# cvg/pixel-perfect-sfm

Hardware: AMD Instinct MI355X
Metric: featuremetric residuals+Jacobians evaluated/sec (1M obs) (higher is better)
Workload: dtype f32 horizontal / f64 vertical+normalisation on f16 patches; 1 GPU; BASELINE.json configs[2]: synthetic 200 cams / 200000 points / 1000000 obs featuremetric BA residual+Jacobian evaluation, 128-ch fp16 16x16 patches, SIMPLE_RADIAL, fused six-scalar Jacobian reduction; n_obs=1000000, channels=128, patch=16, obs_per_gpu=1000000, partition=none

## Files before the change

pixel-perfect-sfm_amd/csrc/pxr_ba_gram.hip:

```cpp
#include <hip/hip_runtime.h>

#include <algorithm>

#include "pxr_ba_solve.h"
#include "pxr_device.h"
#include "pxr_gram.h"
#include "pxr_internal.h"

namespace pxr {

constexpr int GC_STRIDE = IG_GDOUBLES + 16;

struct GramArgs {
  pxr_ba_view v;
  const void* arena; const int32_t* corners; const double* scales;
  int H, W, l2_normalize;
  double* G;
  int2* cell;
  int* dirty;
  const double* r2;
  double* rec;
};

template <typename ST, int C>
__global__ __launch_bounds__(64) void k_gram_build(const GramArgs a) {
// ... 26 lines not shown
      if (2 * lane < C) rr = *reinterpret_cast<const double2*>(a.v.d_refs + (size_t)p * C + 2 * lane);
      return j;
    };
    auto build = [&](const GramTexels<ST, C>& tx, const double2& rr, int slot, int j) {
      if (2 * lane < C) *reinterpret_cast<double2*>(&refbuf[slot][2 * lane]) = rr;
      __syncthreads();
      double* g = a.G + (size_t)(base + j) * GC_STRIDE;
      gram_contract<ST, C>(tx, refbuf[slot], g, g + IG_GDOUBLES);
    };
    GramTexels<ST, C> t0, t1, t2;
    int s0 = take(t0, rr0), s1 = take(t1, rr1), s2 = take(t2, rr2);
    while (true) {
      if (s0 < 0) break;
      build(t0, rr0, 0, s0); s0 = take(t0, rr0);
      if (s1 < 0) break;
      build(t1, rr1, 1, s1); s1 = take(t1, rr1);
      if (s2 < 0) break;
      build(t2, rr2, 2, s2); s2 = take(t2, rr2);
    }
  }
}

template <bool FIRST>
__device__ __forceinline__ void gram_eval_eight(const GramArgs& a, double* S, int64_t i, int nq, int lane) {
  const int q = lane >> 3, sub = lane & 7, ri = sub >> 1, ci = 2 * (sub & 1);
  constexpr int NT = (8 * GC_STRIDE / 2 + 63) / 64, PER = GC_STRIDE / 2;
  static_assert(NT * 64 == 8 * PER, "the last request stays inside the buffer");
  const int n2 = nq * PER;
#pragma unroll
  for (int j = 0; j < NT; ++j) {
    const int e = min(lane + 64 * j, n2 - 1);
    const double2* src;
    if (FIRST) {
      src = reinterpret_cast<const double2*>(a.G + (size_t)__shfl((int)i, 0) * GC_STRIDE) + e;
    } else {
      const int64_t oi = __shfl((int)i, 8 * (e / PER));
      src = reinterpret_cast<const double2*>(a.G + (size_t)oi * GC_STRIDE) + e % PER;
    }
    __builtin_amdgcn_global_load_lds((const __attribute__((address_space(1))) void*)src,
                                     (__attribute__((address_space(3))) void*)(S + 2 * 64 * j), 16, 0, 0);
  }
  const int img = a.v.d_obs_image[i];
  const int pt = a.v.d_obs_point[i];
  const int64_t pidx = a.v.d_obs_patch[i];
  int2 cached = make_int2(0, 0);
  if (FIRST) cached = a.cell[i];
  const int cam = a.v.d_image_camera[img];
  double qv[4], t[3], X[3], k[PXR_KPAD];
#pragma unroll
  for (int j = 0; j < 4; ++j) qv[j] = a.v.d_qvec[4 * (size_t)img + j];
#pragma unroll
  for (int j = 0; j < 3; ++j) { t[j] = a.v.d_tvec[3 * (size_t)img + j]; X[j] = a.v.d_xyz[3 * (size_t)pt + j]; }
#pragma unroll
  for (int j = 0; j < PXR_KPAD; ++j) k[j] = a.v.d_cam_params[(size_t)cam * PXR_KPAD + j];
  const double sx = a.scales[2 * pidx], sy = a.scales[2 * pidx + 1];
  const double cx = (double)a.corners[2 * pidx], cy = (double)a.corners[2 * pidx + 1];
  const double r2 = a.r2[pt];
  double x, y;
  world_to_pixel(a.v.d_cam_model[cam], k, qv, t, X, x, y);
  const double u = x * sx - 0.5 - cx, v = y * sy - 0.5 - cy;
  const double rf = floor(v), cf = floor(u);
  const int row = texel_index(rf, a.H), col = texel_index(cf, a.W);
  const bool miss = FIRST && (cached.x != row || cached.y != col);
  if (FIRST && q < nq && sub == 0) {
    a.dirty[i] = miss ? 1 : 0;
    if (miss) a.cell[i] = make_int2(row, col);
  }
  double wu[4], dwu[4], wv[4], dwv[4];
  catmull_rom_weights(u - cf, wu, dwu);
  catmull_rom_weights(v - rf, wv, dwv);
  __builtin_amdgcn_s_waitcnt(0x0f70);
  __syncthreads();
  if (q >= nq || miss) return;
  const double* Gq = S + (size_t)q * GC_STRIDE;
  double ya[3], yb[3];
  gram_rows_times_weights(Gq, sub, wu, dwu, wv, dwv, ya, yb);
  const double2 d2 = *reinterpret_cast<const double2*>(Gq + IG_GDOUBLES + 2 * sub);
  const double wvo = pick4(wv, ri), dwvo = pick4(dwv, ri);
  const double wua = ci == 0 ? wu[0] : wu[2], wub = ci == 0 ? wu[1] : wu[3];
  const double dwua = ci == 0 ? dwu[0] : dwu[2], dwub = ci == 0 ? dwu[1] : dwu[3];
  const double oma = wvo * wua, omb = wvo * wub, omca = wvo * dwua, omcb = wvo * dwub, omra = dwvo * wua, omrb = dwvo * wub;
  const double Sgg = row8_sum(fma(oma, ya[0], omb * yb[0])), Sgc = row8_sum(fma(oma, ya[1], omb * yb[1]));
  const double Sgr = row8_sum(fma(oma, ya[2], omb * yb[2]));
  const double Scc = row8_sum(fma(omca, ya[1], omcb * yb[1])), Scr = row8_sum(fma(omca, ya[2], omcb * yb[2]));
  const double Srr = row8_sum(fma(omra, ya[2], omrb * yb[2]));
  const double Sfd = row8_sum(fma(oma, d2.x, omb * d2.y)), Scd = row8_sum(fma(omca, d2.x, omcb * d2.y));
  const double Srd = row8_sum(fma(omra, d2.x, omrb * d2.y));
  if (sub != 0) return;
  double s, gcc, gcr, grr, bc, br;
  if (a.l2_normalize) {
    const double ninv = 1.0 / sqrt(Sgg), n2inv = ninv * ninv;
    const double pc = Sgc * n2inv, pr = Sgr * n2inv;
    s = 1.0 - 2.0 * Sfd * ninv + r2;
    gcc = (Scc - Sgc * pc) * n2inv; gcr = (Scr - Sgc * pr) * n2inv; grr = (Srr - Sgr * pr) * n2inv;
    bc = -(Scd - Sfd * pc) * ninv; br = -(Srd - Sfd * pr) * ninv;
  } else {
    s = Sgg - 2.0 * Sfd + r2;
    gcc = Scc; gcr = Scr; grr = Srr; bc = Sgc - Scd; br = Sgr - Srd;
  }
  if (s < 0.0) s = 0.0;
  double2* out = reinterpret_cast<double2*>(a.rec + (size_t)i * PXR_OBS_REC);
  out[0] = make_double2(s, gcc * sx * sx);
  out[1] = make_double2(gcr * sx * sy, grr * sy * sy);
  out[2] = make_double2(bc * sx, br * sy);
  out[3] = make_double2(x, y);
}

__global__ __launch_bounds__(64) void k_gram_eval(const GramArgs a) {
  __shared__ __align__(16) double S[8 * GC_STRIDE];
  const int lane = threadIdx.x;
  const int64_t o0 = (int64_t)blockIdx.x * 8;
  const int nq = (int)min<int64_t>(8, a.v.n_obs - o0);
  if (nq <= 0) return;
  gram_eval_eight<true>(a, S, o0 + min(lane >> 3, nq - 1), nq, lane);
}

__global__ __launch_bounds__(64) void k_gram_eval_dirty(const GramArgs a) {
  __shared__ __align__(16) double S[8 * GC_STRIDE];
  const int lane = threadIdx.x;
  const int64_t base = (int64_t)blockIdx.x * 64, n = a.v.n_obs;
  unsigned long long todo = __ballot(base + lane < n && a.dirty[min(base + lane, n - 1)] != 0);
#pragma clang loop unroll(disable)
  while (todo != 0ull) {
    const int nq = min(8, __popcll(todo));
    unsigned long long m = todo;
    for (int t = min(lane >> 3, nq - 1); t > 0; --t) m &= m - 1ull;
    const int64_t i = base + __ffsll((long long)m) - 1;
    gram_eval_eight<false>(a, S, i, nq, lane);
    for (int t = 0; t < nq; ++t) todo &= todo - 1ull;
    __syncthreads();
  }
}

__global__ __launch_bounds__(256) void k_gram_count_dirty(int64_t n, const int* __restrict__ dirty, int* __restrict__ count) {
  const int64_t i = (int64_t)blockIdx.x * blockDim.x + threadIdx.x;
  const unsigned long long m = __ballot(i < n && dirty[min(i, n - 1)] != 0);
  if ((threadIdx.x & 63) == 0 && m != 0ull) atomicAdd(count, __popcll(m));
}

__global__ __launch_bounds__(256) void k_gram_r2(int64_t n_pts, int C, const double* __restrict__ refs, double* __restrict__ r2) {
  const int64_t t = (int64_t)blockIdx.x * blockDim.x + threadIdx.x;
  const int64_t p = t >> 4;
  const int sub = (int)(t & 15);
  double acc = 0.0;
  if (p < n_pts)
    for (int ch = sub; ch < C; ch += 16) { const double d = refs[(size_t)p * C + ch]; acc = fma(d, d, acc); }
  acc = row16_sum(acc);
  if (p < n_pts && sub == 0) r2[p] = acc;
}

__global__ __launch_bounds__(256) void k_gram_invalidate(int64_t n, int2* __restrict__ cell) {
  const int64_t i = (int64_t)blockIdx.x * blockDim.x + threadIdx.x;
  if (i < n) cell[i] = make_int2(-1000000, -1000000);
}
// ... 30 lines not shown
  }
  gram_layout(ctx->d_gram, n, np, out, &need);
  hipStream_t st = ctx->stream;
  hipLaunchKernelGGL(k_gram_invalidate, dim3((unsigned)((n + 255) / 256)), dim3(256), 0, st, n, static_cast<int2*>(out->cell));
  hipLaunchKernelGGL(k_gram_r2, dim3((unsigned)((np * 16 + 255) / 256)), dim3(256), 0, st, np, arena->C, view->d_refs, out->r2);
  return hip_check(hipGetLastError(), "Gram-matrix cache set-up");
}

int gram_build_flagged(pxr_ctx* ctx, pxr_arena* arena, const pxr_ba_view* v, const GramCache& gc) {
  GramArgs a;
  a.v = *v;
  a.arena = arena->d_data; a.corners = arena->d_corners; a.scales = arena->d_scales;
  a.H = arena->H; a.W = arena->W; a.l2_normalize = 0;
  a.G = gc.G; a.cell = static_cast<int2*>(gc.cell); a.dirty = gc.list; a.r2 = gc.r2; a.rec = nullptr;
  const int64_t n = v->n_obs;
  const unsigned build_grid = (unsigned)std::min<int64_t>((n + 63) / 64, (int64_t)ctx->num_cus * 16);
#define GRAM_BUILD(ST, CC) hipLaunchKernelGGL((k_gram_build<ST, CC>), dim3(build_grid), dim3(64), 0, ctx->stream, a)
  if (arena->dtype == PXR_F16) { if (arena->C == 128) GRAM_BUILD(_Float16, 128); else GRAM_BUILD(_Float16, 64); }
  else { if (arena->C == 128) GRAM_BUILD(float, 128); else GRAM_BUILD(float, 64); }
#undef GRAM_BUILD
  return hip_check(hipGetLastError(), "Gram-matrix build");
}

int gram_evaluate(pxr_ctx* ctx, pxr_arena* arena, const pxr_ba_view* v, const pxr_interp_cfg* cfg, const GramCache& gc, double* rec) {
  GramArgs a;
  a.v = *v;
  a.arena = arena->d_data; a.corners = arena->d_corners; a.scales = arena->d_scales;
  a.H = arena->H; a.W = arena->W; a.l2_normalize = cfg->l2_normalize;
  a.G = gc.G; a.cell = static_cast<int2*>(gc.cell); a.dirty = gc.list; a.r2 = gc.r2; a.rec = rec;
  hipStream_t st = ctx->stream;
  const int64_t n = v->n_obs;
  hipLaunchKernelGGL(k_gram_eval, dim3((unsigned)((n + 7) / 8)), dim3(64), 0, st, a);
  const unsigned build_grid = (unsigned)std::min<int64_t>((n + 63) / 64, (int64_t)ctx->num_cus * 16);
#define GRAM_BUILD(ST, CC) hipLaunchKernelGGL((k_gram_build<ST, CC>), dim3(build_grid), dim3(64), 0, st, a)
  if (arena->dtype == PXR_F16) { if (arena->C == 128) GRAM_BUILD(_Float16, 128); else GRAM_BUILD(_Float16, 64); }
  else { if (arena->C == 128) GRAM_BUILD(float, 128); else GRAM_BUILD(float, 64); }
#undef GRAM_BUILD
  hipLaunchKernelGGL(k_gram_eval_dirty, dim3((unsigned)((n + 63) / 64)), dim3(64), 0, st, a);
  return hip_check(hipGetLastError(), "Gram-matrix evaluation");
}

}

extern "C" int pxr_ba_eval_gram(pxr_ctx* ctx, pxr_arena* arena, const pxr_ba_view* view, const pxr_interp_cfg* cfg, int reset,
                                double* d_rec, int32_t* h_rebuilt) {
  using namespace pxr;
  PXR_REQUIRE(ctx && arena && view && cfg && d_rec, "pxr_ba_eval_gram: NULL argument");
  PXR_REQUIRE(gram_eval_supported(arena, view), "pxr_ba_eval_gram: needs feature patches of 128 / 64 channels in fp16 / fp32 storage and reference descriptors");
  PXR_HIP(hipSetDevice(ctx->device));
  GramCache gc;
  size_t need = 0;
  gram_layout(ctx->d_gram, view->n_obs, view->n_points, &gc, &need);
  if (reset || ctx->gram_bytes < need) {
    if (int rc = gram_eval_prepare(ctx, arena, view, &gc)) return rc;
  }
  if (int rc = gram_evaluate(ctx, arena, view, cfg, gc, d_rec)) return rc;
  if (h_rebuilt) {
    PXR_HIP(hipMemsetAsync(gc.count, 0, sizeof(int), ctx->stream));
    hipLaunchKernelGGL(k_gram_count_dirty, dim3((unsigned)((view->n_obs + 255) / 256)), dim3(256), 0, ctx->stream, view->n_obs, gc.list, gc.count);
    PXR_HIP(hipMemcpyAsync(h_rebuilt, gc.count, sizeof(int32_t), hipMemcpyDeviceToHost, ctx->stream));
    PXR_HIP(hipStreamSynchronize(ctx->stream));
  }
// ... 4 lines not shown
```

pixel-perfect-sfm_amd/csrc/pxr_ba_solve.h:

```cpp
#pragma once
#include <hip/hip_runtime.h>

#include <functional>

#include "pixsfm_hip.h"

namespace pxr {

struct SolveDev {
  pxr_ba_view v;
  const int* pose_off; const int* pose_dim; const int* tmask;
  const int* intr_off; const int* intr_dim; const int* cmask;
  const int* pt_var;
  const double* scale_c;
  const double* scale_p;
  int n_c; int DC; int LS;
  int ldS;
};

struct ImgChunk { int img; int64_t begin, end; };

__device__ __forceinline__ int col_index(const SolveDev& d, int img, int cam, int a) {
  const int pd = d.pose_dim[img];
  return a < pd ? d.pose_off[img] + a : d.intr_off[cam] + (a - pd);
}

__device__ __forceinline__ void y_row(const double* __restrict__ W, const double* __restrict__ T, int64_t i, int a, int DC,
                                      int64_t pt, double& y0, double& y1, double& y2) {
  const double* Wi = W + ((size_t)i * DC + a) * 3;
  const double* Tp = T + 6 * (size_t)pt;
  const double w0 = Wi[0], w1 = Wi[1], w2 = Wi[2];
  y0 = w0 * Tp[0] + w1 * Tp[1] + w2 * Tp[2];
  y1 = w0 * Tp[1] + w1 * Tp[3] + w2 * Tp[4];
  y2 = w0 * Tp[2] + w1 * Tp[4] + w2 * Tp[5];
}

__device__ __forceinline__ double wave_sum(double v) {
  for (int off = 32; off > 0; off >>= 1) v += __shfl_xor(v, off);
  return v;
}

}
```

pixel-perfect-sfm_amd/csrc/pxr_ba_solve.hip:

```cpp
#include <hip/hip_runtime.h>

#include <algorithm>
#include <chrono>
#include <cmath>
#include <cstdlib>
#include <cstring>
#include <limits>
#include <thread>
#include <vector>

#include "pxr_ba_pcg.h"
#include "pxr_ba_solve.h"
#include "pxr_device.h"
#include "pxr_internal.h"

namespace pxr {


constexpr int JAC_THREADS = 128;

__global__ __launch_bounds__(JAC_THREADS) void k_jac(const SolveDev d, const double* __restrict__ rec,
                                                     pxr_loss loss, double* __restrict__ L, double* __restrict__ W) {
  extern __shared__ double jstage[];
  const int lane = threadIdx.x & 63, wave = threadIdx.x >> 6;
  const int LS = d.LS, W3 = 3 * d.DC, WS = W3 + 1;
  double* Lw = jstage + (size_t)wave * 64 * (LS + WS);
  double* Ww = Lw + (size_t)64 * LS;
  const int64_t i0 = (int64_t)blockIdx.x * blockDim.x + wave * 64;
  const int64_t i = i0 + lane;
  const int n_valid = (int)min((int64_t)64, d.v.n_obs - i0);
  if (i < d.v.n_obs) {
  const int img = d.v.d_obs_image[i], pt = d.v.d_obs_point[i], cam = d.v.d_image_camera[img];
  double q[4], t[3], X[3], k[PXR_KPAD];
#pragma unroll
  for (int j = 0; j < 4; ++j) q[j] = d.v.d_qvec[4 * (size_t)img + j];
#pragma unroll
  for (int j = 0; j < 3; ++j) { t[j] = d.v.d_tvec[3 * (size_t)img + j]; X[j] = d.v.d_xyz[3 * (size_t)pt + j]; }
#pragma unroll
  for (int j = 0; j < PXR_KPAD; ++j) k[j] = d.v.d_cam_params[(size_t)cam * PXR_KPAD + j];
  const int model = d.v.d_cam_model[cam];
  double x, y, A[2][3], Pq[2][4], PX[2][3], Pk[2][PXR_KPAD];
  world_to_pixel_jac(model, k, q, t, X, x, y, A, Pq, PX, Pk);

  const double* r = rec + (size_t)i * PXR_OBS_REC;
  const double s = r[0], gxx = r[1], gxy = r[2], gyy = r[3], bx = r[4], by = r[5];
// ... 51 lines not shown
    for (int a = 0; a < 3; ++a) {
      if ((tm >> a) & 1) continue;
      const double sc = d.scale_c[po + col];
      put(col, A[0][a] * sc, A[1][a] * sc);
      ++col;
    }
  }
  if (d.intr_dim[cam] > 0) {
    const int io = d.intr_off[cam], cm = d.cmask[cam], K = camera_num_params(model);
    int kc = 0;
#pragma unroll
    for (int a = 0; a < PXR_KPAD; ++a) {
      if (a >= K || ((cm >> a) & 1)) continue;
      const double sc = d.scale_c[io + kc];
      put(col, Pk[0][a] * sc, Pk[1][a] * sc);
      ++col; ++kc;
    }
  }
  for (; col < d.DC; ++col) put(col, 0.0, 0.0);
  }
  __threadfence_block();
  __builtin_amdgcn_wave_barrier();
  if (n_valid <= 0) return;
  double* Lg = L + (size_t)i0 * LS;
  for (int x = lane; x < n_valid * LS; x += 64) Lg[x] = Lw[x];
  double* Wg = W + (size_t)i0 * W3;
  for (int x = lane; x < n_valid * W3; x += 64) { const int o = x / W3; Wg[x] = Ww[o * WS + (x - o * W3)]; }
}

__global__ __launch_bounds__(256) void k_point(const SolveDev d, const int64_t* __restrict__ pt_ptr,
                                               const int64_t* __restrict__ pt_obs,
                                               const double* __restrict__ L, double* __restrict__ V,
                                               double* __restrict__ gp) {
  const int64_t p = (int64_t)blockIdx.x * blockDim.x + threadIdx.x;
  if (p >= d.v.n_points) return;
  double v[6] = {0, 0, 0, 0, 0, 0}, g[3] = {0, 0, 0};
  for (int64_t o = pt_ptr[p]; o < pt_ptr[p + 1]; ++o) {
    const double* Lo = L + (size_t)pt_obs[o] * d.LS;
    const double m00 = Lo[0], m01 = Lo[1], m11 = Lo[2], b0 = Lo[3], b1 = Lo[4];
    const double e0[3] = {Lo[5], Lo[6], Lo[7]}, e1[3] = {Lo[8], Lo[9], Lo[10]};
    double me0[3], me1[3];
#pragma unroll
    for (int j = 0; j < 3; ++j) { me0[j] = m00 * e0[j] + m01 * e1[j]; me1[j] = m01 * e0[j] + m11 * e1[j]; }
    v[0] += e0[0] * me0[0] + e1[0] * me1[0];
    v[1] += e0[0] * me0[1] + e1[0] * me1[1];
    v[2] += e0[0] * me0[2] + e1[0] * me1[2];
    v[3] += e0[1] * me0[1] + e1[1] * me1[1];
    v[4] += e0[1] * me0[2] + e1[1] * me1[2];
    v[5] += e0[2] * me0[2] + e1[2] * me1[2];
#pragma unroll
    for (int j = 0; j < 3; ++j) g[j] += e0[j] * b0 + e1[j] * b1;
  }
#pragma unroll
  for (int j = 0; j < 6; ++j) V[6 * p + j] = v[j];
#pragma unroll
  for (int j = 0; j < 3; ++j) gp[3 * p + j] = g[j];
}

constexpr int IMG_BATCH = 128;

__global__ __launch_bounds__(256) void k_img(const SolveDev d, const ImgChunk* __restrict__ chunks,
                                             const int64_t* __restrict__ img_obs,
                                             const double* __restrict__ L, double* __restrict__ U,
                                             double* __restrict__ gc, int block_form, double det_scale,
                                             double* __restrict__ chunk_trace, double* __restrict__ kpart, int ne_max) {
  extern __shared__ double stage[];
  const ImgChunk ch = chunks[blockIdx.x];
  const int img = ch.img, cam = d.v.d_image_camera[img];
  const int dc = d.pose_dim[img] + d.intr_dim[cam];
  if (dc == 0) { if (threadIdx.x == 0 && chunk_trace) chunk_trace[blockIdx.x] = 0.0; return; }
  const int LS = d.LS;
  double* red = stage + (size_t)IMG_BATCH * LS;
  const int NP = dc * (dc + 1) / 2, NE = NP + dc;
  const int slices = 256 / NE;
  const int e = threadIdx.x % NE, sl = threadIdx.x / NE;
  int a = 0, b = 0;
  const bool is_g = e >= NP;
  if (is_g) { a = e - NP; }
  else { int rem = e; a = 0; while (rem >= dc - a) { rem -= dc - a; ++a; } b = a + rem; }
// ... 822 lines not shown
      if (!on || a.wanted <= a.cap) return;
      (void)hipDeviceSynchronize();
      if (ctx->d_solve_arena) (void)hipFree(ctx->d_solve_arena);
      ctx->d_solve_arena = nullptr; ctx->solve_arena_bytes = 0;
      const size_t want = a.wanted + a.wanted / 16 + (1u << 20);
      if (hipMalloc(&ctx->d_solve_arena, want) == hipSuccess) ctx->solve_arena_bytes = want;
      else { (void)hipGetLastError(); ctx->d_solve_arena = nullptr; }
    }
  } arena_scope(ctx);
  const bool setup_verbose = std::getenv("PXR_VERBOSE") != nullptr;
  auto setup_mark = [&](const char* what) {
    if (setup_verbose)
      fprintf(stderr, "[pxr_ba_solve] setup: %-28s at %.2f ms\n", what,
              std::chrono::duration<double, std::milli>(std::chrono::steady_clock::now() - t_setup0).count());
  };
  const int64_t n_obs = view->n_obs, n_pts = view->n_points;
  const int n_img = view->n_images, n_cam = view->n_cameras;

  std::vector<int32_t> obs_image, obs_point, image_camera(n_img), cam_model(n_cam);
  std::vector<int64_t> img_cnt(n_img + 1, 0), pt_cnt;
  DevBuf<unsigned long long> d_cnt;
  DevBuf<int> d_flags;
  bool device_lists = n_img <= SORT_MAX_IMAGES && std::getenv("PXR_BA_SETUP_HOST") == nullptr;
  PXR_HIP(hipMemcpyAsync(image_camera.data(), view->d_image_camera, 4 * n_img, hipMemcpyDeviceToHost, st));
  PXR_HIP(hipMemcpyAsync(cam_model.data(), view->d_cam_model, 4 * n_cam, hipMemcpyDeviceToHost, st));
  setup_mark("camera tables read");
  if (device_lists) {
    int h_flags[2] = {0, 0};
    RC(d_cnt.alloc((size_t)n_img + 1 + (size_t)n_pts + 1 + 1)); RC(d_flags.alloc(2));
    setup_mark("counter buffers");
    PXR_HIP(hipMemsetAsync(d_cnt.p, 0, sizeof(unsigned long long) * d_cnt.n, st));
    PXR_HIP(hipMemsetAsync(d_flags.p, 0, sizeof(int) * 2, st));
    hipLaunchKernelGGL(k_count_indices, dim3((unsigned)((n_obs + COUNT_CHUNK - 1) / COUNT_CHUNK)), dim3(256), sizeof(unsigned int) * n_img, st, n_obs, view->d_obs_image,
                       view->d_obs_point, n_img, n_pts, d_cnt.p, d_cnt.p + n_img + 1, d_flags.p);
    static_assert(sizeof(unsigned long long) == sizeof(int64_t), "counter width");
    PXR_HIP(hipMemcpyAsync(img_cnt.data(), d_cnt.p, sizeof(int64_t) * (n_img + 1), hipMemcpyDeviceToHost, st));
    PXR_HIP(hipMemcpyAsync(h_flags, d_flags.p, sizeof(int) * 2, hipMemcpyDeviceToHost, st));
    PXR_HIP(hipStreamSynchronize(st));
    PXR_REQUIRE(h_flags[0] == 0, "pxr_ba_solve: an observation references an image / point out of range");
    if (h_flags[1]) {
      device_lists = false;
      std::fill(img_cnt.begin(), img_cnt.end(), 0);
    }
  }
  if (!device_lists) {
    pt_cnt.assign(n_pts + 1, 0);
// ... 83 lines not shown
    for (int i = 0; i < n_img; ++i) {
      const int c = image_camera[i];
      const bool joint = cam_users[c] == 1 && intr_dim[c] > 0;
      if (pose_dim[i] == 0 && !joint) continue;
      const int g = open_group();
      add_cols(g, pose_off[i], pose_dim[i]);
      if (joint) add_cols(g, intr_off[c], intr_dim[c]);
    }
    for (int c = 0; c < n_cam; ++c)
      if (cam_users[c] != 1 && intr_dim[c] > 0) add_cols(open_group(), intr_off[c], intr_dim[c]);
    for (int c = 0; c < n_c; ++c) PXR_REQUIRE(col_group[c].x >= 0, "pxr_ba_solve: internal: column %d in no preconditioner block", c);
  }
  setup_mark("host structure (CSR, chunks)");
  DevBuf<int> d_pose_off, d_pose_dim, d_tmask, d_intr_off, d_intr_dim, d_cmask, d_pt_var;
  DevBuf<int64_t> d_img_obs, d_pt_ptr, d_pt_obs;
  DevBuf<ImgChunk> d_chunks, d_schur_chunks;
  DevBuf<int4> d_obs_cols, d_so;
  DevBuf<int> d_part_obs;
  RC(d_pose_off.upload(pose_off, st)); RC(d_pose_dim.upload(pose_dim, st)); RC(d_tmask.upload(tmask, st));
  RC(d_intr_off.upload(intr_off, st)); RC(d_intr_dim.upload(intr_dim, st)); RC(d_cmask.upload(cmask, st));
  RC(d_chunks.upload(chunks, st));
  DevBuf<uint8_t> d_pt_const;
  DevBuf<unsigned long long> d_pt_part;
  unsigned long long h_n_pvar = 0;
  if (!device_lists) { RC(d_pt_var.upload(pt_var, st)); RC(d_pt_ptr.upload(pt_cnt, st)); }
  if (device_lists) {
    const int n_parts = (int)((n_pts + PT_SCAN_CHUNK - 1) / PT_SCAN_CHUNK);
    unsigned long long* const d_pt_cnt = d_cnt.p + n_img + 1;
    RC(d_pt_var.alloc(n_pts)); RC(d_pt_ptr.alloc((size_t)n_pts + 1)); RC(d_pt_const.alloc(n_pts)); RC(d_pt_part.alloc(n_parts));
    PXR_HIP(hipMemcpyAsync(d_pt_const.p, h_point_const, (size_t)n_pts, hipMemcpyHostToDevice, st));
    hipLaunchKernelGGL(k_pt_scan_partials, dim3(n_parts), dim3(256), 0, st, n_pts, (const unsigned long long*)d_pt_cnt, d_pt_part.p);
    hipLaunchKernelGGL(k_pt_scan_apply, dim3(n_parts), dim3(256), 0, st, n_pts, (const unsigned long long*)d_pt_cnt, (const unsigned long long*)d_pt_part.p,
                       (const uint8_t*)d_pt_const.p, d_pt_ptr.p, d_pt_var.p, d_pt_cnt + n_pts + 1);
    PXR_HIP(hipMemcpyAsync(&h_n_pvar, d_pt_cnt + n_pts + 1, sizeof(h_n_pvar), hipMemcpyDeviceToHost, st));
    RC(d_img_obs.alloc(n_obs)); RC(d_pt_obs.alloc(n_obs));
    hipLaunchKernelGGL(k_iota, dim3(nblk(n_obs)), dim3(256), 0, st, n_obs, d_pt_obs.p);
    DevBuf<int64_t> d_img_ptr;
    DevBuf<int> d_hist;
    const int n_chunks = (int)((n_obs + SORT_CHUNK - 1) / SORT_CHUNK);
    RC(d_img_ptr.upload(img_cnt, st)); RC(d_hist.alloc((size_t)n_chunks * n_img));
    hipLaunchKernelGGL(k_sort_hist, dim3(n_chunks), dim3(256), sizeof(int) * n_img, st, n_obs, view->d_obs_image, n_img, d_hist.p);
    hipLaunchKernelGGL(k_sort_offsets, dim3((n_img + 255) / 256), dim3(256), 0, st, n_img, n_chunks, d_img_ptr.p, d_hist.p);
    hipLaunchKernelGGL(k_sort_scatter, dim3(n_chunks), dim3(256), sizeof(int) * (n_img + 256), st, n_obs, view->d_obs_image, n_img,
                       d_hist.p, d_img_obs.p);
    LAUNCH_CHECK("observation-list kernels");
    setup_mark("list kernels launched");
    PXR_HIP(hipStreamSynchronize(st));
    setup_mark("list kernels done");
    n_pvar = (int64_t)h_n_pvar;
    PXR_REQUIRE(n_c > 0 || n_pvar > 0, "pxr_ba_solve: every parameter block is constant");
  } else {
    RC(d_img_obs.upload(img_obs, st)); RC(d_pt_obs.upload(pt_obs, st));
  }
  RC(d_schur_chunks.upload(schur_chunks, st));
  RC(d_obs_cols.alloc(n_obs)); RC(d_so.alloc(n_obs)); RC(d_part_obs.alloc(n_obs));
  hipLaunchKernelGGL(k_build_descriptors, dim3(nblk(n_obs)), dim3(256), 0, st, n_obs, view->d_obs_image, view->d_obs_point,
                     view->d_image_camera, d_pt_obs.p, d_img_obs.p, d_pt_ptr.p, d_pt_var.p, d_pose_off.p, d_pose_dim.p,
                     d_intr_off.p, d_intr_dim.p, d_obs_cols.p, d_part_obs.p, d_so.p);
  LAUNCH_CHECK("k_build_descriptors");
  setup_mark("index uploads");
  const size_t nc1 = n_c ? n_c : 1;
  DevBuf<double> L, V, gp, Vd0, T, W, U, S , gcd , damp_c, scale_c, scale_p,
      delta_c, delta_p, rec_a, rec_b, q1, t1, k1, X1, scal;
  RC(L.alloc((size_t)n_obs * LS)); RC(V.alloc((size_t)n_pts * 6)); RC(gp.alloc((size_t)n_pts * 3));
  RC(Vd0.alloc((size_t)n_pts * 3)); RC(T.alloc((size_t)n_pts * 6));
  RC(W.alloc((size_t)n_obs * DC * 3));
  RC(U.alloc(iterative ? (size_t)n_img * DC * DC : nc1 * nc1)); RC(S.alloc(iterative ? 1 : (nc1 + 1) * (nc1 + 1)));
// ... 138 lines not shown
  RC(chunk_trace.alloc(chunks.size() + 1));
  auto det_scale_for = [](double md, double cost_now) {
    const double bound = 8.0 * std::max({md, std::sqrt(2.0 * md * std::max(cost_now, 0.0)), 1e-300});
    return std::ldexp(1.0, 62 - (int)std::ceil(std::log2(bound)));
  };
  double lin_md = 1.0;
  bool gram_cache = !geom && ctx->gram_cache && gram_eval_supported(arena, view) && cfg->use_float_simd == 0;
  bool gram_inner = !geom && opt->use_inner_iterations != 0 && arena->dtype != PXR_F64 && (arena->C == 128 || arena->C == 64) && !getenv("PXR_INNER_OLD") &&
                    !getenv("PXR_INNER_PACKED") && cfg->use_float_simd == 0;
  for (int c = 0; c < n_cam; ++c) gram_inner = gram_inner && cam_model[c] <= PXR_OPENCV;
  bool inner_cache = gram_inner && gram_eval_supported(arena, view) && !getenv("PXR_INNER_NO_CACHE");
  GramCache gram;
  if ((gram_cache || inner_cache) && gram_eval_prepare(ctx, arena, view, &gram) != PXR_OK) {
    gram_cache = false; inner_cache = false;
    (void)set_error(PXR_OK, "");
  }
  bool geom_ext = false;
  for (int c = 0; c < n_cam; ++c) geom_ext = geom_ext || cam_model[c] > PXR_OPENCV;
  setup_mark("Gram-matrix cache prepared");
  bool gram_warm = false;
  int n_evaluations = 0;
  bool cur_is_exact = true;
  auto evaluate = [&](const pxr_ba_view& v, double* rec) -> int {
    if (geom) RC(geom_eval(ctx, &v, d_obs_xy, rec, nullptr));
    else if (gram_cache && n_evaluations > 0) { RC(gram_evaluate(ctx, arena, &v, cfg, gram, rec)); gram_warm = true; }
    else RC(ba_eval_with_cost(ctx, arena, &v, cfg, 1, rec, nullptr, nullptr, nullptr, nullptr, nullptr));
    ++n_evaluations;
    hipLaunchKernelGGL(k_cost_limbs, dim3(1024), dim3(256), 0, st, (const double*)rec, n_obs, *loss, slimb.p + 0 * PXR_LIMBS);
    LAUNCH_CHECK("cost");
    return PXR_OK;
  };
  double lin_scale = 0.0;
  auto linearize = [&](const double* rec) -> int {
    hipLaunchKernelGGL(k_jac, dim3((unsigned)((n_obs + JAC_THREADS - 1) / JAC_THREADS)), dim3(JAC_THREADS),
                       sizeof(double) * (JAC_THREADS / 64) * 64 * (LS + 3 * DC + 1), st, dv, rec, *loss, L.p, W.p);
    hipLaunchKernelGGL(k_point, dim3(nblk(n_pts)), dim3(256), 0, st, dv, d_pt_ptr.p, d_pt_obs.p, L.p, V.p, gp.p);
    PXR_HIP(hipMemsetAsync(U.p, 0, sizeof(double) * U.n, st));
    PXR_HIP(hipMemsetAsync(gcd.p, 0, sizeof(double) * gcd.n, st));
    if (n_c > 0 && !chunks.empty()) {
      hipLaunchKernelGGL(k_img, dim3((unsigned)chunks.size()), dim3(256), sizeof(double) * ((size_t)IMG_BATCH * LS + 256), st, dv,
                         d_chunks.p, d_img_obs.p, L.p, U.p, gc, iterative ? 1 : 0, lin_scale, lin_scale != 0.0 ? chunk_trace.p : (double*)nullptr,
                         det_iter ? det_kpart.p : (double*)nullptr, det_ne_max);
      if (det_iter) {
        RC(pcg_blocks_from_partials(st, dv, d_kchunk_ptr.p, det_kpart.p, det_ne_max, U.p, det_gimg.p, d_col_ent_ptr.p, d_col_ent.p, diagU, gc));
        LAUNCH_CHECK("linearize kernels");
        RC(ar(gcd.p, 2 * (int64_t)nc1));
        return PXR_OK;
      }
      if (lin_scale != 0.0) {
        hipLaunchKernelGGL(k_diag_and_trace, dim3(1), dim3(1024), 0, st, n_c, (const double*)U.p, diagU, (const double*)chunk_trace.p, (int)chunks.size(),
                           reinterpret_cast<long long*>(gcd.p + 2 * nc1));
        RC(ar_i64(reinterpret_cast<long long*>(gcd.p), 2 * (int64_t)nc1 + PXR_LIMBS));
        hipLaunchKernelGGL(k_finish_and_stats, dim3(1), dim3(1024), 0, st, n_c, 2 * (int)nc1, gcd.p, lin_scale,
                           reinterpret_cast<const long long*>(gcd.p + 2 * nc1), lin_stats.p);
        LAUNCH_CHECK("linearize kernels");
        return PXR_OK;
      }
      if (iterative) RC(pcg_diag_from_blocks(st, dv, U.p, diagU));
      else hipLaunchKernelGGL(k_extract_diag, dim3(nblk(n_c)), dim3(256), 0, st, n_c, U.p, diagU);
// ... 379 lines not shown
```

Measured before the change: 1.467 billion residual_blocks/s.

## Pipeline Gram evaluation, fuse loss cost into eval, and fold point sums into k_jac

Replaces the one-block-per-eight-observations Gram evaluation with a persistent, double-buffered kernel that prefetches the next group's Gram rows and camera/point parameters while the current group is projected and reduced. The robust-loss cost is accumulated inside the evaluation and dirty kernels, so the separate cost pass over the records is no longer launched. Point Hessian and gradient sums for points whose observations all sit in one 64-observation window are computed inside k_jac, and the k_point pass only handles the listed straddling points. The change adds register pressure and extra setup (a straddler list and a host readback), and it assumes the point-ordered observation layout keeps most points inside one window.

```diff
diff --git a/pixel-perfect-sfm_amd/csrc/pxr_ba_gram.hip b/pixel-perfect-sfm_amd/csrc/pxr_ba_gram.hip
--- a/pixel-perfect-sfm_amd/csrc/pxr_ba_gram.hip
+++ b/pixel-perfect-sfm_amd/csrc/pxr_ba_gram.hip
@@ -1,6 +1,8 @@
 #include <hip/hip_runtime.h>
 
 #include <algorithm>
+#include <cstdlib>
+#include <cstring>
 
 #include "pxr_ba_solve.h"
 #include "pxr_device.h"
@@ -73,8 +75,7 @@
 }
 
 template <bool FIRST>
-__device__ __forceinline__ void gram_eval_eight(const GramArgs& a, double* S, int64_t i, int nq, int lane) {
-  const int q = lane >> 3, sub = lane & 7, ri = sub >> 1, ci = 2 * (sub & 1);
+__device__ __forceinline__ void gram_request(const GramArgs& a, double* S, int64_t i, int nq, int lane) {
   constexpr int NT = (8 * GC_STRIDE / 2 + 63) / 64, PER = GC_STRIDE / 2;
   static_assert(NT * 64 == 8 * PER, "the last request stays inside the buffer");
   const int n2 = nq * PER;
@@ -91,38 +92,68 @@
     __builtin_amdgcn_global_load_lds((const __attribute__((address_space(1))) void*)src,
                                      (__attribute__((address_space(3))) void*)(S + 2 * 64 * j), 16, 0, 0);
   }
-  const int img = a.v.d_obs_image[i];
-  const int pt = a.v.d_obs_point[i];
-  const int64_t pidx = a.v.d_obs_patch[i];
-  int2 cached = make_int2(0, 0);
-  if (FIRST) cached = a.cell[i];
-  const int cam = a.v.d_image_camera[img];
-  double qv[4], t[3], X[3], k[PXR_KPAD];
-#pragma unroll
-  for (int j = 0; j < 4; ++j) qv[j] = a.v.d_qvec[4 * (size_t)img + j];
-#pragma unroll
-  for (int j = 0; j < 3; ++j) { t[j] = a.v.d_tvec[3 * (size_t)img + j]; X[j] = a.v.d_xyz[3 * (size_t)pt + j]; }
-#pragma unroll
-  for (int j = 0; j < PXR_KPAD; ++j) k[j] = a.v.d_cam_params[(size_t)cam * PXR_KPAD + j];
-  const double sx = a.scales[2 * pidx], sy = a.scales[2 * pidx + 1];
-  const double cx = (double)a.corners[2 * pidx], cy = (double)a.corners[2 * pidx + 1];
-  const double r2 = a.r2[pt];
-  double x, y;
-  world_to_pixel(a.v.d_cam_model[cam], k, qv, t, X, x, y);
-  const double u = x * sx - 0.5 - cx, v = y * sy - 0.5 - cy;
+}
+
+struct GramObs { int img, pt, cam; int64_t pidx; int2 cached; };
+struct GramParams { double qv[4], t[3], X[3], k[PXR_KPAD], sx, sy, cx, cy, r2; int model; };
+struct GramProj { double x, y, sx, sy, r2, wu[4], dwu[4], wv[4], dwv[4]; bool miss; };
+
+template <bool FIRST>
+__device__ __forceinline__ void gram_load_obs(const GramArgs& a, int64_t i, GramObs& o) {
+  o.img = a.v.d_obs_image[i];
+  o.pt = a.v.d_obs_point[i];
+  o.pidx = a.v.d_obs_patch[i];
+  o.cached = make_int2(0, 0);
+  if (FIRST) o.cached = a.cell[i];
+}
+__device__ __forceinline__ void gram_load_params(const GramArgs& a, const GramObs& o, GramParams& p) {
+#pragma unroll
+  for (int j = 0; j < 4; ++j) p.qv[j] = a.v.d_qvec[4 * (size_t)o.img + j];
+#pragma unroll
+  for (int j = 0; j < 3; ++j) { p.t[j] = a.v.d_tvec[3 * (size_t)o.img + j]; p.X[j] = a.v.d_xyz[3 * (size_t)o.pt + j]; }
+#pragma unroll
+  for (int j = 0; j < PXR_KPAD; ++j) p.k[j] = a.v.d_cam_params[(size_t)o.cam * PXR_KPAD + j];
+  p.sx = a.scales[2 * o.pidx]; p.sy = a.scales[2 * o.pidx + 1];
+  p.cx = (double)a.corners[2 * o.pidx]; p.cy = (double)a.corners[2 * o.pidx + 1];
+  p.r2 = a.r2[o.pt];
+  p.model = a.v.d_cam_model[o.cam];
+}
+
+__device__ __forceinline__ void gram_copy_params(GramParams& d, const GramParams& p) {
+#pragma unroll
+  for (int j = 0; j < 4; ++j) d.qv[j] = p.qv[j];
+#pragma unroll
+  for (int j = 0; j < 3; ++j) { d.t[j] = p.t[j]; d.X[j] = p.X[j]; }
+#pragma unroll
+  for (int j = 0; j < PXR_KPAD; ++j) d.k[j] = p.k[j];
+  d.sx = p.sx; d.sy = p.sy; d.cx = p.cx; d.cy = p.cy; d.r2 = p.r2; d.model = p.model;
+}
+
+template <bool FIRST>
+__device__ __forceinline__ void gram_project(const GramArgs& a, int64_t i, int nq, int lane, int2 cached, const GramParams& p,
+                                             GramProj& pr) {
+  const int q = lane >> 3, sub = lane & 7;
+  world_to_pixel(p.model, p.k, p.qv, p.t, p.X, pr.x, pr.y);
+  const double u = pr.x * p.sx - 0.5 - p.cx, v = pr.y * p.sy - 0.5 - p.cy;
   const double rf = floor(v), cf = floor(u);
   const int row = texel_index(rf, a.H), col = texel_index(cf, a.W);
-  const bool miss = FIRST && (cached.x != row || cached.y != col);
+  pr.miss = FIRST && (cached.x != row || cached.y != col);
   if (FIRST && q < nq && sub == 0) {
-    a.dirty[i] = miss ? 1 : 0;
-    if (miss) a.cell[i] = make_int2(row, col);
-  }
-  double wu[4], dwu[4], wv[4], dwv[4];
-  catmull_rom_weights(u - cf, wu, dwu);
-  catmull_rom_weights(v - rf, wv, dwv);
-  __builtin_amdgcn_s_waitcnt(0x0f70);
-  __syncthreads();
-  if (q >= nq || miss) return;
+    a.dirty[i] = pr.miss ? 1 : 0;
+    if (pr.miss) a.cell[i] = make_int2(row, col);
+  }
+  catmull_rom_weights(u - cf, pr.wu, pr.dwu);
+  catmull_rom_weights(v - rf, pr.wv, pr.dwv);
+  pr.sx = p.sx; pr.sy = p.sy; pr.r2 = p.r2;
+}
+
+__device__ __forceinline__ bool gram_record(const GramArgs& a, const double* S, int64_t i, int nq, int lane, const GramProj& pr,
+                                            double& s_out) {
+  const int q = lane >> 3, sub = lane & 7, ri = sub >> 1, ci = 2 * (sub & 1);
+  s_out = 0.0;
+  if (q >= nq || pr.miss) return false;
+  const double (&wu)[4] = pr.wu; const double (&dwu)[4] = pr.dwu; const double (&wv)[4] = pr.wv; const double (&dwv)[4] = pr.dwv;
+  const double sx = pr.sx, sy = pr.sy, r2 = pr.r2, x = pr.x, y = pr.y;
   const double* Gq = S + (size_t)q * GC_STRIDE;
   double ya[3], yb[3];
   gram_rows_times_weights(Gq, sub, wu, dwu, wv, dwv, ya, yb);
@@ -137,14 +168,14 @@
   const double Srr = row8_sum(fma(omra, ya[2], omrb * yb[2]));
   const double Sfd = row8_sum(fma(oma, d2.x, omb * d2.y)), Scd = row8_sum(fma(omca, d2.x, omcb * d2.y));
   const double Srd = row8_sum(fma(omra, d2.x, omrb * d2.y));
-  if (sub != 0) return;
+  if (sub != 0) return false;
   double s, gcc, gcr, grr, bc, br;
   if (a.l2_normalize) {
     const double ninv = 1.0 / sqrt(Sgg), n2inv = ninv * ninv;
-    const double pc = Sgc * n2inv, pr = Sgr * n2inv;
+    const double pc = Sgc * n2inv, pr_ = Sgr * n2inv;
     s = 1.0 - 2.0 * Sfd * ninv + r2;
-    gcc = (Scc - Sgc * pc) * n2inv; gcr = (Scr - Sgc * pr) * n2inv; grr = (Srr - Sgr * pr) * n2inv;
-    bc = -(Scd - Sfd * pc) * ninv; br = -(Srd - Sfd * pr) * ninv;
+    gcc = (Scc - Sgc * pc) * n2inv; gcr = (Scr - Sgc * pr_) * n2inv; grr = (Srr - Sgr * pr_) * n2inv;
+    bc = -(Scd - Sfd * pc) * ninv; br = -(Srd - Sfd * pr_) * ninv;
   } else {
     s = Sgg - 2.0 * Sfd + r2;
     gcc = Scc; gcr = Scr; grr = Srr; bc = Sgc - Scd; br = Sgr - Srd;
@@ -155,6 +186,37 @@
   out[1] = make_double2(gcr * sx * sy, grr * sy * sy);
   out[2] = make_double2(bc * sx, br * sy);
   out[3] = make_double2(x, y);
+  s_out = s;
+  return true;
+}
+
+struct GramCost {
+  Limbs l;
+  long long bad = 0;
+  __device__ __forceinline__ void add(const pxr_loss& loss, double s) {
+    double rho[3];
+    loss_eval(loss.type, loss.a, 1.0, s, rho);
+    const double c = 0.5 * rho[0];
+    const bool ok = fabs(c) < 0x1p60;
+    bad += ok ? 0 : 1;
+    if (ok) l.add(c);
+  }
+  __device__ __forceinline__ Limbs total() const { Limbs t = l; t.q[4] += bad; return t; }
+};
+
+template <bool FIRST>
+__device__ __forceinline__ bool gram_eval_eight(const GramArgs& a, double* S, int64_t i, int nq, int lane, double& s_out) {
+  gram_request<FIRST>(a, S, i, nq, lane);
+  GramObs o;
+  GramParams p;
+  GramProj pr;
+  gram_load_obs<FIRST>(a, i, o);
+  o.cam = a.v.d_image_camera[o.img];
+  gram_load_params(a, o, p);
+  gram_project<FIRST>(a, i, nq, lane, o.cached, p, pr);
+  __builtin_amdgcn_s_waitcnt(0x0f70);
+  __syncthreads();
+  return gram_record(a, S, i, nq, lane, pr, s_out);
 }
 
 __global__ __launch_bounds__(64) void k_gram_eval(const GramArgs a) {
@@ -163,24 +225,77 @@
   const int64_t o0 = (int64_t)blockIdx.x * 8;
   const int nq = (int)min<int64_t>(8, a.v.n_obs - o0);
   if (nq <= 0) return;
-  gram_eval_eight<true>(a, S, o0 + min(lane >> 3, nq - 1), nq, lane);
-}
-
-__global__ __launch_bounds__(64) void k_gram_eval_dirty(const GramArgs a) {
+  double s;
+  gram_eval_eight<true>(a, S, o0 + min(lane >> 3, nq - 1), nq, lane, s);
+}
+
+__global__ __launch_bounds__(64, 2) void k_gram_eval_pipe(const GramArgs a, const pxr_loss loss, long long* __restrict__ cost_slot) {
+  __shared__ __align__(16) double S0[8 * GC_STRIDE];
+  __shared__ __align__(16) double S1[8 * GC_STRIDE];
+  __shared__ long long lsh[PXR_LIMBS];
+  const int lane = threadIdx.x, q = lane >> 3;
+  const int64_t n = a.v.n_obs, n_trips = (n + 7) / 8, step = gridDim.x;
+  auto obs_of = [&](int64_t trip) { return min(trip * 8 + q, n - 1); };
+  auto nq_of = [&](int64_t trip) { return (int)min<int64_t>(8, n - trip * 8); };
+  GramCost cost;
+  int64_t trip = blockIdx.x;
+  if (trip < n_trips) {
+    GramObs o0, o1, o2, o3;
+    GramParams pa, pb;
+    gram_load_obs<true>(a, obs_of(trip), o0);
+    gram_load_obs<true>(a, obs_of(trip + step), o1);
+    gram_load_obs<true>(a, obs_of(trip + 2 * step), o2);
+    o0.cam = a.v.d_image_camera[o0.img];
+    o1.cam = a.v.d_image_camera[o1.img];
+    gram_load_params(a, o0, pa);
+    int2 cached = o0.cached;
+    gram_request<true>(a, S0, obs_of(trip), nq_of(trip), lane);
+    auto stage = [&](double* Sc, double* Sn, const GramParams& pc, GramParams& pn) __attribute__((always_inline)) -> bool {
+      const bool has_next = trip + step < n_trips;
+      __builtin_amdgcn_s_waitcnt(0x0f70);
+      __syncthreads();
+      if (has_next) gram_request<true>(a, Sn, obs_of(trip + step), nq_of(trip + step), lane);
+      gram_load_params(a, o1, pn);
+      o2.cam = a.v.d_image_camera[o2.img];
+      gram_load_obs<true>(a, obs_of(trip + 3 * step), o3);
+      const int64_t i = obs_of(trip);
+      const int nq = nq_of(trip);
+      GramProj pr;
+      gram_project<true>(a, i, nq, lane, cached, pc, pr);
+      double s;
+      if (gram_record(a, Sc, i, nq, lane, pr, s) && cost_slot != nullptr) cost.add(loss, s);
+      if (!has_next) return false;
+      __syncthreads();
+      cached = o1.cached; o1 = o2; o2 = o3;
+      trip += step;
+      return true;
+    };
+    while (stage(S0, S1, pa, pb) && stage(S1, S0, pb, pa)) {}
+  }
+  if (cost_slot != nullptr) limbs_block_add(cost.total(), cost_slot, lsh);
+}
+
+__global__ __launch_bounds__(64) void k_gram_eval_dirty(const GramArgs a, const pxr_loss loss, long long* __restrict__ cost_slot) {
   __shared__ __align__(16) double S[8 * GC_STRIDE];
+  __shared__ long long lsh[PXR_LIMBS];
   const int lane = threadIdx.x;
-  const int64_t base = (int64_t)blockIdx.x * 64, n = a.v.n_obs;
-  unsigned long long todo = __ballot(base + lane < n && a.dirty[min(base + lane, n - 1)] != 0);
+  const int64_t n = a.v.n_obs;
+  GramCost cost;
+  for (int64_t base = (int64_t)blockIdx.x * 64; base < n; base += (int64_t)gridDim.x * 64) {
+    unsigned long long todo = __ballot(base + lane < n && a.dirty[min(base + lane, n - 1)] != 0);
 #pragma clang loop unroll(disable)
-  while (todo != 0ull) {
-    const int nq = min(8, __popcll(todo));
-    unsigned long long m = todo;
-    for (int t = min(lane >> 3, nq - 1); t > 0; --t) m &= m - 1ull;
-    const int64_t i = base + __ffsll((long long)m) - 1;
-    gram_eval_eight<false>(a, S, i, nq, lane);
-    for (int t = 0; t < nq; ++t) todo &= todo - 1ull;
-    __syncthreads();
-  }
+    while (todo != 0ull) {
+      const int nq = min(8, __popcll(todo));
+      unsigned long long m = todo;
+      for (int t = min(lane >> 3, nq - 1); t > 0; --t) m &= m - 1ull;
+      const int64_t i = base + __ffsll((long long)m) - 1;
+      double s;
+      if (gram_eval_eight<false>(a, S, i, nq, lane, s) && cost_slot != nullptr) cost.add(loss, s);
+      for (int t = 0; t < nq; ++t) todo &= todo - 1ull;
+      __syncthreads();
+    }
+  }
+  if (cost_slot != nullptr) limbs_block_add(cost.total(), cost_slot, lsh);
 }
 
 __global__ __launch_bounds__(256) void k_gram_count_dirty(int64_t n, const int* __restrict__ dirty, int* __restrict__ count) {
@@ -257,7 +372,20 @@
   return hip_check(hipGetLastError(), "Gram-matrix build");
 }
 
-int gram_evaluate(pxr_ctx* ctx, pxr_arena* arena, const pxr_ba_view* v, const pxr_interp_cfg* cfg, const GramCache& gc, double* rec) {
+static unsigned gram_pipe_grid(pxr_ctx* ctx, int64_t n_trips) {
+  static int per_cu = 0;
+  if (per_cu == 0) {
+    int nb = 0;
+    if (hipOccupancyMaxActiveBlocksPerMultiprocessor(&nb, k_gram_eval_pipe, 64, 0) != hipSuccess || nb < 1) { (void)hipGetLastError(); nb = 7; }
+    per_cu = nb;
+  }
+  int64_t g = (int64_t)per_cu * ctx->num_cus;
+  if (const char* e = getenv("PXR_GRAM_EVAL_WAVES")) { const long w = atol(e); if (w > 0) g = w; }
+  return (unsigned)std::max<int64_t>(1, std::min(g, n_trips));
+}
+
+int gram_evaluate_front(pxr_ctx* ctx, pxr_arena* arena, const pxr_ba_view* v, const pxr_interp_cfg* cfg, const GramCache& gc, double* rec,
+                        const pxr_loss* loss, long long* cost_slot, bool legacy) {
   GramArgs a;
   a.v = *v;
   a.arena = arena->d_data; a.corners = arena->d_corners; a.scales = arena->d_scales;
@@ -265,14 +393,24 @@
   a.G = gc.G; a.cell = static_cast<int2*>(gc.cell); a.dirty = gc.list; a.r2 = gc.r2; a.rec = rec;
   hipStream_t st = ctx->stream;
   const int64_t n = v->n_obs;
-  hipLaunchKernelGGL(k_gram_eval, dim3((unsigned)((n + 7) / 8)), dim3(64), 0, st, a);
+  pxr_loss ls;
+  memset(&ls, 0, sizeof(ls));
+  if (legacy || loss == nullptr) cost_slot = nullptr;
+  if (cost_slot != nullptr) ls = *loss;
+  if (legacy) hipLaunchKernelGGL(k_gram_eval, dim3((unsigned)((n + 7) / 8)), dim3(64), 0, st, a);
+  else hipLaunchKernelGGL(k_gram_eval_pipe, dim3(gram_pipe_grid(ctx, (n + 7) / 8)), dim3(64), 0, st, a, ls, cost_slot);
   const unsigned build_grid = (unsigned)std::min<int64_t>((n + 63) / 64, (int64_t)ctx->num_cus * 16);
 #define GRAM_BUILD(ST, CC) hipLaunchKernelGGL((k_gram_build<ST, CC>), dim3(build_grid), dim3(64), 0, st, a)
   if (arena->dtype == PXR_F16) { if (arena->C == 128) GRAM_BUILD(_Float16, 128); else GRAM_BUILD(_Float16, 64); }
   else { if (arena->C == 128) GRAM_BUILD(float, 128); else GRAM_BUILD(float, 64); }
 #undef GRAM_BUILD
-  hipLaunchKernelGGL(k_gram_eval_dirty, dim3((unsigned)((n + 63) / 64)), dim3(64), 0, st, a);
+  const unsigned dirty_grid = cost_slot != nullptr ? build_grid : (unsigned)((n + 63) / 64);
+  hipLaunchKernelGGL(k_gram_eval_dirty, dim3(dirty_grid), dim3(64), 0, st, a, ls, cost_slot);
   return hip_check(hipGetLastError(), "Gram-matrix evaluation");
+}
+
+int gram_evaluate(pxr_ctx* ctx, pxr_arena* arena, const pxr_ba_view* v, const pxr_interp_cfg* cfg, const GramCache& gc, double* rec) {
+  return gram_evaluate_front(ctx, arena, v, cfg, gc, rec, nullptr, nullptr, lm_front_legacy());
 }
 
 }
diff --git a/pixel-perfect-sfm_amd/csrc/pxr_ba_solve.h b/pixel-perfect-sfm_amd/csrc/pxr_ba_solve.h
--- a/pixel-perfect-sfm_amd/csrc/pxr_ba_solve.h
+++ b/pixel-perfect-sfm_amd/csrc/pxr_ba_solve.h
@@ -1,6 +1,7 @@
 #pragma once
 #include <hip/hip_runtime.h>
 
+#include <cstdlib>
 #include <functional>
 
 #include "pixsfm_hip.h"
@@ -40,4 +41,9 @@
   return v;
 }
 
+inline bool lm_front_legacy() { const char* e = std::getenv("PXR_LM_FRONT_LEGACY"); return e != nullptr && e[0] != '\0' && e[0] != '0'; }
+struct GramCache;
+int gram_evaluate_front(pxr_ctx* ctx, pxr_arena* arena, const pxr_ba_view* v, const pxr_interp_cfg* cfg, const GramCache& gc, double* rec,
+                        const pxr_loss* loss, long long* cost_slot, bool legacy);
+
 }
diff --git a/pixel-perfect-sfm_amd/csrc/pxr_ba_solve.hip b/pixel-perfect-sfm_amd/csrc/pxr_ba_solve.hip
--- a/pixel-perfect-sfm_amd/csrc/pxr_ba_solve.hip
+++ b/pixel-perfect-sfm_amd/csrc/pxr_ba_solve.hip
@@ -19,8 +19,26 @@
 
 constexpr int JAC_THREADS = 128;
 
+__device__ __forceinline__ void point_accumulate(const double* Lo, double (&v)[6], double (&g)[3]) {
+  const double m00 = Lo[0], m01 = Lo[1], m11 = Lo[2], b0 = Lo[3], b1 = Lo[4];
+  const double e0[3] = {Lo[5], Lo[6], Lo[7]}, e1[3] = {Lo[8], Lo[9], Lo[10]};
+  double me0[3], me1[3];
+#pragma unroll
+  for (int j = 0; j < 3; ++j) { me0[j] = m00 * e0[j] + m01 * e1[j]; me1[j] = m01 * e0[j] + m11 * e1[j]; }
+  v[0] += e0[0] * me0[0] + e1[0] * me1[0];
+  v[1] += e0[0] * me0[1] + e1[0] * me1[1];
+  v[2] += e0[0] * me0[2] + e1[0] * me1[2];
+  v[3] += e0[1] * me0[1] + e1[1] * me1[1];
+  v[4] += e0[1] * me0[2] + e1[1] * me1[2];
+  v[5] += e0[2] * me0[2] + e1[2] * me1[2];
+#pragma unroll
+  for (int j = 0; j < 3; ++j) g[j] += e0[j] * b0 + e1[j] * b1;
+}
+
 __global__ __launch_bounds__(JAC_THREADS) void k_jac(const SolveDev d, const double* __restrict__ rec,
-                                                     pxr_loss loss, double* __restrict__ L, double* __restrict__ W) {
+                                                     pxr_loss loss, double* __restrict__ L, double* __restrict__ W,
+                                                     const int64_t* __restrict__ pt_ptr, double* __restrict__ V,
+                                                     double* __restrict__ gp) {
   extern __shared__ double jstage[];
   const int lane = threadIdx.x & 63, wave = threadIdx.x >> 6;
   const int LS = d.LS, W3 = 3 * d.DC, WS = W3 + 1;
@@ -118,6 +136,18 @@
   __threadfence_block();
   __builtin_amdgcn_wave_barrier();
   if (n_valid <= 0) return;
+  if (pt_ptr != nullptr && i < d.v.n_obs) {
+    const int64_t p = d.v.d_obs_point[i];
+    const int64_t b = pt_ptr[p], e = pt_ptr[p + 1];
+    if (b == i && e <= i0 + 64) {
+      double v[6] = {0, 0, 0, 0, 0, 0}, g[3] = {0, 0, 0};
+      for (int64_t o = b; o < e; ++o) point_accumulate(Lw + (size_t)(o - i0) * LS, v, g);
+#pragma unroll
+      for (int j = 0; j < 6; ++j) V[6 * p + j] = v[j];
+#pragma unroll
+      for (int j = 0; j < 3; ++j) gp[3 * p + j] = g[j];
+    }
+  }
   double* Lg = L + (size_t)i0 * LS;
   for (int x = lane; x < n_valid * LS; x += 64) Lg[x] = Lw[x];
   double* Wg = W + (size_t)i0 * W3;
@@ -127,30 +157,23 @@
 __global__ __launch_bounds__(256) void k_point(const SolveDev d, const int64_t* __restrict__ pt_ptr,
                                                const int64_t* __restrict__ pt_obs,
                                                const double* __restrict__ L, double* __restrict__ V,
-                                               double* __restrict__ gp) {
+                                               double* __restrict__ gp, const int* __restrict__ list, int64_t count) {
+  const int64_t t = (int64_t)blockIdx.x * blockDim.x + threadIdx.x;
+  if (t >= count) return;
+  const int64_t p = list != nullptr ? (int64_t)list[t] : t;
+  double v[6] = {0, 0, 0, 0, 0, 0}, g[3] = {0, 0, 0};
+  for (int64_t o = pt_ptr[p]; o < pt_ptr[p + 1]; ++o) point_accumulate(L + (size_t)pt_obs[o] * d.LS, v, g);
+#pragma unroll
+  for (int j = 0; j < 6; ++j) V[6 * p + j] = v[j];
+#pragma unroll
+  for (int j = 0; j < 3; ++j) gp[3 * p + j] = g[j];
+}
+__global__ __launch_bounds__(256) void k_point_straddlers(int64_t n_points, const int64_t* __restrict__ pt_ptr, int* __restrict__ list,
+                                                          int* __restrict__ count) {
   const int64_t p = (int64_t)blockIdx.x * blockDim.x + threadIdx.x;
-  if (p >= d.v.n_points) return;
-  double v[6] = {0, 0, 0, 0, 0, 0}, g[3] = {0, 0, 0};
-  for (int64_t o = pt_ptr[p]; o < pt_ptr[p + 1]; ++o) {
-    const double* Lo = L + (size_t)pt_obs[o] * d.LS;
-    const double m00 = Lo[0], m01 = Lo[1], m11 = Lo[2], b0 = Lo[3], b1 = Lo[4];
-    const double e0[3] = {Lo[5], Lo[6], Lo[7]}, e1[3] = {Lo[8], Lo[9], Lo[10]};
-    double me0[3], me1[3];
-#pragma unroll
-    for (int j = 0; j < 3; ++j) { me0[j] = m00 * e0[j] + m01 * e1[j]; me1[j] = m01 * e0[j] + m11 * e1[j]; }
-    v[0] += e0[0] * me0[0] + e1[0] * me1[0];
-    v[1] += e0[0] * me0[1] + e1[0] * me1[1];
-    v[2] += e0[0] * me0[2] + e1[0] * me1[2];
-    v[3] += e0[1] * me0[1] + e1[1] * me1[1];
-    v[4] += e0[1] * me0[2] + e1[1] * me1[2];
-    v[5] += e0[2] * me0[2] + e1[2] * me1[2];
-#pragma unroll
-    for (int j = 0; j < 3; ++j) g[j] += e0[j] * b0 + e1[j] * b1;
-  }
-#pragma unroll
-  for (int j = 0; j < 6; ++j) V[6 * p + j] = v[j];
-#pragma unroll
-  for (int j = 0; j < 3; ++j) gp[3 * p + j] = g[j];
+  if (p >= n_points) return;
+  const int64_t b = pt_ptr[p], e = pt_ptr[p + 1];
+  if (e == b || b / 64 != (e - 1) / 64) list[atomicAdd(count, 1)] = (int)p;
 }
 
 constexpr int IMG_BATCH = 128;
@@ -1019,6 +1042,7 @@
   DevBuf<unsigned long long> d_cnt;
   DevBuf<int> d_flags;
   bool device_lists = n_img <= SORT_MAX_IMAGES && std::getenv("PXR_BA_SETUP_HOST") == nullptr;
+  const bool front_legacy = lm_front_legacy();
   PXR_HIP(hipMemcpyAsync(image_camera.data(), view->d_image_camera, 4 * n_img, hipMemcpyDeviceToHost, st));
   PXR_HIP(hipMemcpyAsync(cam_model.data(), view->d_cam_model, 4 * n_cam, hipMemcpyDeviceToHost, st));
   setup_mark("camera tables read");
@@ -1148,6 +1172,9 @@
   RC(d_chunks.upload(chunks, st));
   DevBuf<uint8_t> d_pt_const;
   DevBuf<unsigned long long> d_pt_part;
+  DevBuf<int> d_straddle;
+  int h_n_straddle = 0;
+  bool jac_point_sums = false;
   unsigned long long h_n_pvar = 0;
   if (!device_lists) { RC(d_pt_var.upload(pt_var, st)); RC(d_pt_ptr.upload(pt_cnt, st)); }
   if (device_lists) {
@@ -1169,6 +1196,14 @@
     hipLaunchKernelGGL(k_sort_offsets, dim3((n_img + 255) / 256), dim3(256), 0, st, n_img, n_chunks, d_img_ptr.p, d_hist.p);
     hipLaunchKernelGGL(k_sort_scatter, dim3(n_chunks), dim3(256), sizeof(int) * (n_img + 256), st, n_obs, view->d_obs_image, n_img,
                        d_hist.p, d_img_obs.p);
+    if (!front_legacy) {
+      static_assert(JAC_THREADS % 64 == 0, "k_jac's wavefront windows are the 64-aligned ones");
+      RC(d_straddle.alloc((size_t)n_pts + 1));
+      PXR_HIP(hipMemsetAsync(d_straddle.p + n_pts, 0, sizeof(int), st));
+      hipLaunchKernelGGL(k_point_straddlers, dim3(nblk(n_pts)), dim3(256), 0, st, n_pts, (const int64_t*)d_pt_ptr.p, d_straddle.p, d_straddle.p + n_pts);
+      PXR_HIP(hipMemcpyAsync(&h_n_straddle, d_straddle.p + n_pts, sizeof(int), hipMemcpyDeviceToHost, st));
+      jac_point_sums = true;
+    }
     LAUNCH_CHECK("observation-list kernels");
     setup_mark("list kernels launched");
     PXR_HIP(hipStreamSynchronize(st));
@@ -1353,19 +1388,26 @@
   int n_evaluations = 0;
   bool cur_is_exact = true;
   auto evaluate = [&](const pxr_ba_view& v, double* rec) -> int {
+    bool cost_done = false;
     if (geom) RC(geom_eval(ctx, &v, d_obs_xy, rec, nullptr));
-    else if (gram_cache && n_evaluations > 0) { RC(gram_evaluate(ctx, arena, &v, cfg, gram, rec)); gram_warm = true; }
+    else if (gram_cache && n_evaluations > 0) {
+      RC(gram_evaluate_front(ctx, arena, &v, cfg, gram, rec, loss, slimb.p + 0 * PXR_LIMBS, front_legacy));
+      gram_warm = true; cost_done = !front_legacy;
+    }
     else RC(ba_eval_with_cost(ctx, arena, &v, cfg, 1, rec, nullptr, nullptr, nullptr, nullptr, nullptr));
     ++n_evaluations;
-    hipLaunchKernelGGL(k_cost_limbs, dim3(1024), dim3(256), 0, st, (const double*)rec, n_obs, *loss, slimb.p + 0 * PXR_LIMBS);
+    if (!cost_done) hipLaunchKernelGGL(k_cost_limbs, dim3(1024), dim3(256), 0, st, (const double*)rec, n_obs, *loss, slimb.p + 0 * PXR_LIMBS);
     LAUNCH_CHECK("cost");
     return PXR_OK;
   };
   double lin_scale = 0.0;
   auto linearize = [&](const double* rec) -> int {
     hipLaunchKernelGGL(k_jac, dim3((unsigned)((n_obs + JAC_THREADS - 1) / JAC_THREADS)), dim3(JAC_THREADS),
-                       sizeof(double) * (JAC_THREADS / 64) * 64 * (LS + 3 * DC + 1), st, dv, rec, *loss, L.p, W.p);
-    hipLaunchKernelGGL(k_point, dim3(nblk(n_pts)), dim3(256), 0, st, dv, d_pt_ptr.p, d_pt_obs.p, L.p, V.p, gp.p);
+                       sizeof(double) * (JAC_THREADS / 64) * 64 * (LS + 3 * DC + 1), st, dv, rec, *loss, L.p, W.p,
+                       jac_point_sums ? (const int64_t*)d_pt_ptr.p : (const int64_t*)nullptr, V.p, gp.p);
+    if (!jac_point_sums) hipLaunchKernelGGL(k_point, dim3(nblk(n_pts)), dim3(256), 0, st, dv, d_pt_ptr.p, d_pt_obs.p, L.p, V.p, gp.p, (const int*)nullptr, n_pts);
+    else if (h_n_straddle > 0) hipLaunchKernelGGL(k_point, dim3(nblk(h_n_straddle)), dim3(256), 0, st, dv, d_pt_ptr.p, d_pt_obs.p, L.p, V.p, gp.p,
+                                                  (const int*)d_straddle.p, (int64_t)h_n_straddle);
     PXR_HIP(hipMemsetAsync(U.p, 0, sizeof(double) * U.n, st));
     PXR_HIP(hipMemsetAsync(gcd.p, 0, sizeof(double) * gcd.n, st));
     if (n_c > 0 && !chunks.empty()) {
```

Result: no change. 1.464 billion residual_blocks/s (-0.2%).
